# cheukwaylee/ORB_SLAM2_detailed_comments

Hardware: AMD Instinct MI355X
Metric: frames/sec ORB extract+match (1000 kp, 640x480) (higher is better)
Workload: dtype u8; 1 GPU; synthetic 640x480 mono stream, nFeatures=1000, 8 levels, scale 1.2, FAST 20/7, extract+match(t vs t-1), batch 1024 frames/GPU resident in HBM, 1 pipelines/GPU; parallelism=single GPU

## Files before the change

orb_slam2_detailed_comments_amd/csrc/orbx_kernels.hip:

```cpp
#include "orbx_device.h"
#include "orbx_inplace.h"
#include "orbx_fast_net.h"
#include "orbx_track.h"
#include "../../include/orbx_pattern_data.h"

#define L0_ROWS 8
#ifndef L0_FF
#define L0_FF 1
#endif
#ifndef RR_FF
#define RR_FF 1
#endif
#define QT_KPT ORBX_QT_KPT
#ifndef QT_DROP_STAGE_A
#define QT_DROP_STAGE_A 1
#endif
#ifndef QT_ONE_SCAN
#define QT_ONE_SCAN 1
#endif
#ifndef QT_REG_SIZE
#define QT_REG_SIZE 1
#endif
#ifndef QT_CENSUS_NODES
#define QT_CENSUS_NODES 1
// ... 1927 lines not shown
                const uint32_t a01 = __builtin_amdgcn_alignbyte(w1, w0, j), a12 = __builtin_amdgcn_alignbyte(w2, w1, j),
                               a23 = __builtin_amdgcn_alignbyte(w3, w2, j);
                hv[j] = __builtin_amdgcn_udot4(a01, KLO, __builtin_amdgcn_udot4(a12, KHI, 0u, false), false);
                hv[4 + j] = __builtin_amdgcn_udot4(a12, KLO, __builtin_amdgcn_udot4(a23, KHI, 0u, false), false);
            }
            uint4 o;
            o.x = hv[0] | (hv[1] << 16);
            o.y = hv[2] | (hv[3] << 16);
            o.z = hv[4] | (hv[5] << 16);
            o.w = hv[6] | (hv[7] << 16);
            *(uint4 *)(hrow + r * DS_HC + 8 * q8) = o;
        }
#endif
        __builtin_amdgcn_fence(__ATOMIC_RELEASE, "wavefront");
        __builtin_amdgcn_wave_barrier();
        __builtin_amdgcn_fence(__ATOMIC_ACQUIRE, "wavefront");
        if (dbg_stop == 3) return;
        const float factorPI = (float)(3.1415926535897932384626433832795 / 180.f);
        const float angle = angle_deg * factorPI;
                const OrbxSinCos sc = orbx_sincosf_pinned(angle);
        const float a = sc.c, b = sc.s;
        const int wvec = (L.pw - 2 * L.org) & ~3;
#if DS_PATTERN_F32
#define DS_PX(t) (((t) & 1) ? patf[(t) >> 1].z : patf[(t) >> 1].x)
#define DS_PY(t) (((t) & 1) ? patf[(t) >> 1].w : patf[(t) >> 1].y)
#else
        const int pw4[4] = {pat.x, pat.y, pat.z, pat.w};
#define DS_PX(t) ((float)(signed char)((pw4[(t) >> 1] >> (16 * ((t) & 1))) & 0xff))
#define DS_PY(t) ((float)(signed char)((pw4[(t) >> 1] >> (16 * ((t) & 1) + 8)) & 0xff))
#endif
        unsigned long long words[4];
        if (x + (DS_R - 3) < wvec) {
#if DS_COLFIRST
            const uint32_t cbias = (uint32_t)(2 * ((DS_R - 3) * DS_VC + (DS_R - 3))) - 0x400000u * (2u * DS_VC) - (0x4B400000u << 1);
#else
            const uint32_t cbias = (uint32_t)(2 * ((DS_R - 3) * DS_HC + (DS_R - 3))) - 0x400000u * (2u * DS_HC) - (0x4B400000u << 1);
#endif
            const uint32_t hbase = (uint32_t)(uintptr_t)(orbx_lds_u16p)hrow + cbias;
            float tv[8];
            float nb = -b;
            asm("" : "+v"(nb));
#pragma unroll
            for (int t0 = 0; t0 < 8; t0 += DS_TAP_BATCH) {
                uint32_t adr[DS_TAP_BATCH], I[DS_TAP_BATCH];
#pragma unroll
                for (int k = 0; k < DS_TAP_BATCH; ++k) {
                    const float px = DS_PX(t0 + k), py = DS_PY(t0 + k);
                    float fy, fx;
                    if (FPM == ORBX_FP_GCC_FMA) {
                        fy = __builtin_fmaf(px, b, py * a);
                        fx = __builtin_fmaf(px, a, py * nb);
                    } else {
                        fy = px * b + py * a;
                        fx = px * a + py * nb;
                    }
                    const uint32_t uy = __float_as_uint(fy + 12582912.0f), ux = __float_as_uint(fx + 12582912.0f);
#if DS_COLFIRST
#if DS_MFMA
                    uint32_t ay = (uy << 1) + hbase;
                    asm("" : "+v"(ay));
                    adr[k] = __umul24(ux, 2u * DS_VC) + ay;
#else
                    adr[k] = __umul24(uy, 2u * DS_VC) + ((ux << 1) + hbase);
#endif
#else
                    adr[k] = __umul24(uy, 2u * DS_HC) + ((ux << 1) + hbase);
                    asm("" : "+v"(adr[k]));
#endif
                }
#if DS_COLFIRST
                orbx_ds_taps<DS_TAP_BATCH>(adr, I);
#else
#pragma unroll
                for (int k = 0; k < DS_TAP_BATCH; ++k) {
                    const orbx_lds_u16p hp = (orbx_lds_u16p)(uintptr_t)adr[k];
                    const uint32_t r0 = hp[3 * DS_HC], r1 = (uint32_t)hp[2 * DS_HC] + hp[4 * DS_HC],
                                   r2 = (uint32_t)hp[1 * DS_HC] + hp[5 * DS_HC], r3 = (uint32_t)hp[0] + hp[6 * DS_HC];
                    I[k] = __umul24(55u, r0) + __umul24(49u, r1) + __umul24(34u, r2) + __umul24(18u, r3);
                }
#endif
#pragma unroll
                for (int k = 0; k < DS_TAP_BATCH; ++k) tv[t0 + k] = __builtin_fminf(__builtin_rintf((float)I[k] * (1.f / 65536.f)), 255.f);
            }
#pragma unroll
            for (int r = 0; r < 4; ++r) words[r] = orbx_ballot(tv[2 * r] < tv[2 * r + 1]);
        } else {
            int tval[8];
#pragma unroll
            for (int t0 = 0; t0 < 8; t0 += DS_TAP_BATCH) {
                uint32_t adr[DS_TAP_BATCH], I[DS_TAP_BATCH];
                int ixs[DS_TAP_BATCH];
#pragma unroll
                for (int k = 0; k < DS_TAP_BATCH; ++k) {
                    const float px = DS_PX(t0 + k), py = DS_PY(t0 + k);
                    float fy, fx;
                    if (FPM == ORBX_FP_GCC_FMA) {
                        fy = __builtin_fmaf(px, b, py * a);
                        fx = __builtin_fmaf(px, a, -(py * b));
                    } else {
                        fy = px * b + py * a;
                        fx = px * a - py * b;
                    }
                    const int iy = (int)__builtin_rintf(fy), ix = (int)__builtin_rintf(fx);
                    ixs[k] = ix;
#if DS_COLFIRST
#if DS_MFMA
                    adr[k] = (uint32_t)(uintptr_t)(orbx_lds_u16p)hrow + 2u * (uint32_t)(__mul24(ix + DS_R - 3, DS_VC) + (iy + DS_R - 3));
#else
                    adr[k] = (uint32_t)(uintptr_t)(orbx_lds_u16p)hrow + 2u * (uint32_t)(__mul24(iy + DS_R - 3, DS_VC) + (ix + DS_R - 3));
#endif
#else
                    adr[k] = (uint32_t)(__mul24(iy + DS_R - 3, DS_HC) + (ix + DS_R - 3));
#endif
                }
#if DS_COLFIRST
                orbx_ds_taps<DS_TAP_BATCH>(adr, I);
#else
#pragma unroll
                for (int k = 0; k < DS_TAP_BATCH; ++k) {
                    const uint16_t *hp = hrow + adr[k];
                    const uint32_t r0 = hp[3 * DS_HC], r1 = (uint32_t)hp[2 * DS_HC] + hp[4 * DS_HC],
                                   r2 = (uint32_t)hp[1 * DS_HC] + hp[5 * DS_HC], r3 = (uint32_t)hp[0] + hp[6 * DS_HC];
                    I[k] = __umul24(55u, r0) + __umul24(49u, r1) + __umul24(34u, r2) + __umul24(18u, r3);
                }
#endif
#pragma unroll
                for (int k = 0; k < DS_TAP_BATCH; ++k) {
                    const uint32_t tie = x + ixs[k] >= wvec ? 1u : ((I[k] >> 16) & 1u);
                    tval[t0 + k] = (int)min((I[k] + 0x7fffu + tie) >> 16, 255u);
                }
            }
#pragma unroll
            for (int r = 0; r < 4; ++r) words[r] = orbx_ballot(tval[2 * r] < tval[2 * r + 1]);
        }
        if (lane < 4) {
            unsigned long long w = lane == 0 ? words[0] : lane == 1 ? words[1] : lane == 2 ? words[2] : words[3];
            *(unsigned long long *)(desc + ((long long)f * cap + oi) * 32 + 8 * lane) = w;
        }
        if (lane == 0) {
            orbx_keypoint kp;
            float fx = (float)x, fy = (float)y;
            if (level != 0) { fx = fx * L.scale; fy = fy * L.scale; }
            kp.x = fx; kp.y = fy;
            kp.size = L.size;
            kp.angle = angle_deg;
            kp.response = (float)(pos >> 24);
            kp.octave = level;
            kp.class_id = -1;
            kps[(long long)f * cap + oi] = kp;
        }
    }
}

#define MT_SPLIT 16
#define MT_WAVES 4
#define MT_QPW(QT) (32 * (QT))
#define MT_QPB(QT) (MT_WAVES * MT_QPW(QT))
#define MT_CHUNK 4096
typedef int mt_v4i __attribute__((ext_vector_type(4)));
typedef int mt_v16i __attribute__((ext_vector_type(16)));
__device__ __forceinline__ uint32_t mt_min2(uint32_t a, uint32_t b) { return a < b ? a : b; }
__device__ __forceinline__ uint32_t mt_max2(uint32_t a, uint32_t b) { return a > b ? a : b; }
template <int QT>
__global__ __launch_bounds__(64 * MT_WAVES, QT == 2 ? 3 : 2) void k_match(const uint8_t *__restrict__ q, const int *__restrict__ nq,
                                                         long long q_stride, const uint8_t *__restrict__ t,
                                                         const int *__restrict__ nt, long long t_stride,
                                                         uint2 *__restrict__ partial, int *__restrict__ best_idx,
                                                         int *__restrict__ best_dist, int *__restrict__ second_dist,
                                                         int out_stride, int nsplit) {
    __shared__ __attribute__((aligned(16))) int s_tk[MT_CHUNK];
    const int lane = threadIdx.x & 63, w = __builtin_amdgcn_readfirstlane(threadIdx.x >> 6), pr = blockIdx.z, sp = blockIdx.y;
    const int NQ = min(nq[pr], out_stride), NT = min(nt[pr], 1 << 20);
    if ((int)blockIdx.x * MT_QPB(QT) >= NQ) return;
    const int r = lane & 31, h = lane >> 5;
    const uint8_t *qp = q + (long long)pr * q_stride;
    const uint8_t *tp = t + (long long)pr * t_stride;
    const int per = ((NT + 31) / 32 + nsplit - 1) / nsplit * 32;
    const int j0 = min(NT, sp * per), j1 = min(NT, j0 + per);
    const int qw = blockIdx.x * MT_QPB(QT) + w * MT_QPW(QT);
    const bool wave_on = qw < NQ;
    mt_v4i bq[QT][8];
    int pq[QT];
#pragma unroll
    for (int c = 0; c < QT; ++c) {
        const int qi = qw + 32 * c + r;
        uint4 v = make_uint4(0, 0, 0, 0);
        if (qi < NQ) v = *(const uint4 *)(qp + (long long)qi * 32 + 16 * h);
        pq[c] = __popc(v.x) + __popc(v.y) + __popc(v.z) + __popc(v.w);
        pq[c] += __shfl_xor(pq[c], 32);
#pragma unroll
        for (int p = 0; p < 8; ++p) {
            bq[c][p][0] = (int)((v.x << (7 - p)) & 0x80808080u);
            bq[c][p][1] = (int)((v.y << (7 - p)) & 0x80808080u);
            bq[c][p][2] = (int)((v.z << (7 - p)) & 0x80808080u);
            bq[c][p][3] = (int)((v.w << (7 - p)) & 0x80808080u);
        }
    }
    uint32_t gbest[QT], gsecond[QT];
#pragma unroll
    for (int c = 0; c < QT; ++c) gbest[c] = gsecond[c] = 0xffffffffu;
    for (int c0 = j0; c0 < j1; c0 += MT_CHUNK) {
        const int c1 = min(j1, c0 + MT_CHUNK), n = c1 - c0, npad = (n + 31) & ~31;
        __syncthreads();
        for (int i = threadIdx.x; i < npad; i += 64 * MT_WAVES) {
            int key = 0x7fffffff;
            if (i < n) {
                const uint4 a = *(const uint4 *)(tp + (long long)(c0 + i) * 32), b = *(const uint4 *)(tp + (long long)(c0 + i) * 32 + 16);
                const int pt = __popc(a.x) + __popc(a.y) + __popc(a.z) + __popc(a.w) + __popc(b.x) + __popc(b.y) + __popc(b.z) + __popc(b.w);
                key = ((pt + 256) << 12) | i;
            }
            s_tk[i] = key;
        }
        __syncthreads();
        if (!wave_on) continue;
        int best[QT], second[QT];
#pragma unroll
        for (int c = 0; c < QT; ++c) best[c] = second[c] = 0x7fffffff;
        const uint8_t *trow = tp + (long long)(c0 + r) * 32 + 16 * h;
        uint4 ta = make_uint4(0, 0, 0, 0);
        if (r < n) ta = *(const uint4 *)trow;
        for (int jt = 0; jt < npad; jt += 32) {
            const uint4 tc = ta;
            ta = make_uint4(0, 0, 0, 0);
            if (jt + 32 + r < n) ta = *(const uint4 *)(trow + (long long)(jt + 32) * 32);
            mt_v16i acc[QT];
            {
                const int4 *kp = (const int4 *)(s_tk + jt + 4 * h);
#pragma unroll
                for (int g = 0; g < 4; ++g) {
                    const int4 k4 = kp[2 * g];
                    acc[0][4 * g] = k4.x; acc[0][4 * g + 1] = k4.y; acc[0][4 * g + 2] = k4.z; acc[0][4 * g + 3] = k4.w;
                }
#pragma unroll
                for (int c = 1; c < QT; ++c) acc[c] = acc[0];
            }
#pragma unroll
            for (int p = 0; p < 8; ++p) {
                mt_v4i a;
                if (p < 6) {
                    a[0] = (int)((tc.x << (6 - p)) & 0x40404040u); a[1] = (int)((tc.y << (6 - p)) & 0x40404040u);
                    a[2] = (int)((tc.z << (6 - p)) & 0x40404040u); a[3] = (int)((tc.w << (6 - p)) & 0x40404040u);
                } else if (p == 6) {
                    a[0] = (int)(tc.x & 0x40404040u); a[1] = (int)(tc.y & 0x40404040u);
                    a[2] = (int)(tc.z & 0x40404040u); a[3] = (int)(tc.w & 0x40404040u);
                } else {
                    a[0] = (int)((tc.x >> 1) & 0x40404040u); a[1] = (int)((tc.y >> 1) & 0x40404040u);
                    a[2] = (int)((tc.z >> 1) & 0x40404040u); a[3] = (int)((tc.w >> 1) & 0x40404040u);
                }
#pragma unroll
                for (int c = 0; c < QT; ++c) acc[c] = __builtin_amdgcn_mfma_i32_32x32x32_i8(a, bq[c][p], acc[c], 0, 0, 0);
            }
#pragma unroll
            for (int i = 0; i < 16; ++i) {
#pragma unroll
                for (int c = 0; c < QT; ++c) {
                    const int kc = acc[c][i];
                    second[c] = max(min(best[c], second[c]), min(max(best[c], second[c]), kc));
                    best[c] = min(best[c], kc);
                }
            }
        }
#pragma unroll
        for (int c = 0; c < QT; ++c) {
            const uint32_t b = best[c] == 0x7fffffff ? 0xffffffffu
                                                     : ((uint32_t)((best[c] >> 12) + pq[c] - 256) << 20) | (uint32_t)(c0 + (best[c] & 4095));
            const uint32_t s2 = second[c] == 0x7fffffff ? 0xffffffffu
                                                        : ((uint32_t)((second[c] >> 12) + pq[c] - 256) << 20) | (uint32_t)(c0 + (second[c] & 4095));
            gsecond[c] = mt_min2(mt_min2(gsecond[c], s2), mt_max2(gbest[c], b));
            gbest[c] = mt_min2(gbest[c], b);
        }
    }
    if (!wave_on) return;
#pragma unroll
    for (int c = 0; c < QT; ++c) {
        const uint32_t ob = (uint32_t)__shfl_xor((int)gbest[c], 32), os = (uint32_t)__shfl_xor((int)gsecond[c], 32);
        const uint32_t second = mt_min2(mt_min2(gsecond[c], os), mt_max2(gbest[c], ob));
        const uint32_t best = mt_min2(gbest[c], ob);
        const int qi = qw + 32 * c + r;
        if (h == 0 && qi < NQ) {
            if (nsplit > 1) {
                partial[((long long)pr * nsplit + sp) * out_stride + qi] = make_uint2(best, second);
            } else {
                const long long o = (long long)pr * out_stride + qi;
                best_idx[o] = best == 0xffffffffu ? -1 : (int)(best & 0xfffffu);
                best_dist[o] = best == 0xffffffffu ? 0x7fffffff : (int)(best >> 20);
                second_dist[o] = second == 0xffffffffu ? 0x7fffffff : (int)(second >> 20);
            }
        }
    }
}

typedef int mt_v8i __attribute__((ext_vector_type(8)));
typedef float mt_v16f __attribute__((ext_vector_type(16)));
#define MT_F4_NONE 0x7f7fffff
#ifndef MT_F4_LB2
#define MT_F4_LB2 3
#endif
#ifndef MT_F4_LB4
#define MT_F4_LB4 2
#endif
#ifndef MT_F4_USE4
#define MT_F4_USE4 1
#endif
template <int QT>
__global__ __launch_bounds__(64 * MT_WAVES, QT == 2 ? MT_F4_LB2 : MT_F4_LB4) void k_match_f4(const uint8_t *__restrict__ q, const int *__restrict__ nq,
                                                         long long q_stride, const uint8_t *__restrict__ t,
                                                         const int *__restrict__ nt, long long t_stride,
                                                         uint2 *__restrict__ partial, int *__restrict__ best_idx,
                                                         int *__restrict__ best_dist, int *__restrict__ second_dist,
                                                         int out_stride, int nsplit) {
    __shared__ __attribute__((aligned(16))) float s_tk[MT_CHUNK];
    const int lane = threadIdx.x & 63, w = __builtin_amdgcn_readfirstlane(threadIdx.x >> 6), pr = blockIdx.z, sp = blockIdx.y;
    const int NQ = min(nq[pr], out_stride), NT = min(nt[pr], 1 << 20);
    if ((int)blockIdx.x * MT_QPB(QT) >= NQ) return;
    const int r = lane & 31, h = lane >> 5;
    const uint8_t *qp = q + (long long)pr * q_stride;
    const uint8_t *tp = t + (long long)pr * t_stride;
    const int per = ((NT + 31) / 32 + nsplit - 1) / nsplit * 32;
    const int j0 = min(NT, sp * per), j1 = min(NT, j0 + per);
    const int qw = blockIdx.x * MT_QPB(QT) + w * MT_QPW(QT);
    const bool wave_on = qw < NQ;
    mt_v4i bq[QT][4];
    int pq[QT];
#pragma unroll
    for (int c = 0; c < QT; ++c) {
        const int qi = qw + 32 * c + r;
        uint4 v = make_uint4(0, 0, 0, 0);
        if (qi < NQ) v = *(const uint4 *)(qp + (long long)qi * 32 + 16 * h);
        pq[c] = __popc(v.x) + __popc(v.y) + __popc(v.z) + __popc(v.w);
        pq[c] += __shfl_xor(pq[c], 32);
        const uint32_t vv[4] = {v.x, v.y, v.z, v.w};
#pragma unroll
        for (int p = 0; p < 4; ++p) {
#pragma unroll
            for (int k = 0; k < 4; ++k) {
                const uint32_t e = (vv[p] >> k) & 0x11111111u;
                bq[c][p][k] = (int)((e << 1) | (e << 2) | (e << 3));
            }
        }
    }
    uint32_t gbest[QT], gsecond[QT];
#pragma unroll
    for (int c = 0; c < QT; ++c) gbest[c] = gsecond[c] = 0xffffffffu;
    for (int c0 = j0; c0 < j1; c0 += MT_CHUNK) {
        const int c1 = min(j1, c0 + MT_CHUNK), n = c1 - c0, npad = (n + 31) & ~31;
        __syncthreads();
        for (int i = threadIdx.x; i < npad; i += 64 * MT_WAVES) {
            float key = __int_as_float(MT_F4_NONE);
            if (i < n) {
                const uint4 a = *(const uint4 *)(tp + (long long)(c0 + i) * 32), b = *(const uint4 *)(tp + (long long)(c0 + i) * 32 + 16);
                const int pt = __popc(a.x) + __popc(a.y) + __popc(a.z) + __popc(a.w) + __popc(b.x) + __popc(b.y) + __popc(b.z) + __popc(b.w);
                key = (float)(((pt + 256) << 12) | i);
            }
            s_tk[i] = key;
        }
        __syncthreads();
        if (!wave_on) continue;
        int best[QT], second[QT];
#pragma unroll
        for (int c = 0; c < QT; ++c) best[c] = second[c] = MT_F4_NONE;
        const uint8_t *trow = tp + (long long)(c0 + r) * 32 + 16 * h;
        uint4 ta = make_uint4(0, 0, 0, 0);
        if (r < n) ta = *(const uint4 *)trow;
        for (int jt = 0; jt < npad; jt += 32) {
            const uint4 tc = ta;
            ta = make_uint4(0, 0, 0, 0);
            if (jt + 32 + r < n) ta = *(const uint4 *)(trow + (long long)(jt + 32) * 32);
            mt_v16f acc[QT];
            {
                const float4 *kp = (const float4 *)(s_tk + jt + 4 * h);
#pragma unroll
                for (int g = 0; g < 4; ++g) {
                    const float4 k4 = kp[2 * g];
                    acc[0][4 * g] = k4.x; acc[0][4 * g + 1] = k4.y; acc[0][4 * g + 2] = k4.z; acc[0][4 * g + 3] = k4.w;
                }
#pragma unroll
                for (int c = 1; c < QT; ++c) acc[c] = acc[0];
            }
            const uint32_t tw[4] = {tc.x, tc.y, tc.z, tc.w};
#pragma unroll
            for (int p = 0; p < 4; ++p) {
                mt_v8i a = {0, 0, 0, 0, 0, 0, 0, 0};
                a[0] = (int)((tw[p] << 2) & 0x44444444u); a[1] = (int)((tw[p] << 1) & 0x44444444u);
                a[2] = (int)(tw[p] & 0x44444444u);        a[3] = (int)((tw[p] >> 1) & 0x44444444u);
#pragma unroll
                for (int c = 0; c < QT; ++c) {
                    mt_v8i b = {0, 0, 0, 0, 0, 0, 0, 0};
                    b[0] = bq[c][p][0]; b[1] = bq[c][p][1]; b[2] = bq[c][p][2]; b[3] = bq[c][p][3];
                    acc[c] = __builtin_amdgcn_mfma_scale_f32_32x32x64_f8f6f4(a, b, acc[c], 4, 4, 0, 137, 0, 127);
                }
            }
#pragma unroll
            for (int i = 0; i < 16; ++i) {
#pragma unroll
                for (int c = 0; c < QT; ++c) {
                    const int kc = __float_as_int(acc[c][i]);
                    second[c] = max(min(best[c], second[c]), min(max(best[c], second[c]), kc));
                    best[c] = min(best[c], kc);
                }
            }
        }
#pragma unroll
        for (int c = 0; c < QT; ++c) {
            const int bk = (int)__int_as_float(best[c]), sk = (int)__int_as_float(second[c]);
            const uint32_t b = best[c] == MT_F4_NONE ? 0xffffffffu
                                                     : ((uint32_t)((bk >> 12) + pq[c] - 256) << 20) | (uint32_t)(c0 + (bk & 4095));
            const uint32_t s2 = second[c] == MT_F4_NONE ? 0xffffffffu
                                                        : ((uint32_t)((sk >> 12) + pq[c] - 256) << 20) | (uint32_t)(c0 + (sk & 4095));
            gsecond[c] = mt_min2(mt_min2(gsecond[c], s2), mt_max2(gbest[c], b));
            gbest[c] = mt_min2(gbest[c], b);
        }
    }
    if (!wave_on) return;
#pragma unroll
    for (int c = 0; c < QT; ++c) {
        const uint32_t ob = (uint32_t)__shfl_xor((int)gbest[c], 32), os = (uint32_t)__shfl_xor((int)gsecond[c], 32);
        const uint32_t second = mt_min2(mt_min2(gsecond[c], os), mt_max2(gbest[c], ob));
        const uint32_t best = mt_min2(gbest[c], ob);
        const int qi = qw + 32 * c + r;
        if (h == 0 && qi < NQ) {
            if (nsplit > 1) {
                partial[((long long)pr * nsplit + sp) * out_stride + qi] = make_uint2(best, second);
            } else {
                const long long o = (long long)pr * out_stride + qi;
                best_idx[o] = best == 0xffffffffu ? -1 : (int)(best & 0xfffffu);
                best_dist[o] = best == 0xffffffffu ? 0x7fffffff : (int)(best >> 20);
                second_dist[o] = second == 0xffffffffu ? 0x7fffffff : (int)(second >> 20);
            }
        }
    }
}

__global__ __launch_bounds__(64) void k_match_valu(const uint8_t *__restrict__ q, const int *__restrict__ nq,
                                                         long long q_stride, const uint8_t *__restrict__ t,
                                                         const int *__restrict__ nt, long long t_stride,
                                                         uint2 *__restrict__ partial, int out_stride, int nsplit) {
    const int lane = threadIdx.x, pr = blockIdx.z, sp = blockIdx.y;
    const int NQ = min(nq[pr], out_stride), NT = min(nt[pr], 1 << 20);
    const int qw = blockIdx.x * 128;
    if (qw >= NQ) return;
    const int qi0 = qw + lane, qi1 = qi0 + 64;
    const uint4 *qp = (const uint4 *)(q + (long long)pr * q_stride);
    const uint4 *tp = (const uint4 *)(t + (long long)pr * t_stride);
    uint4 qa0 = make_uint4(0, 0, 0, 0), qb0 = qa0, qa1 = qa0, qb1 = qa0;
    if (qi0 < NQ) { qa0 = qp[2 * qi0]; qb0 = qp[2 * qi0 + 1]; }
    if (qi1 < NQ) { qa1 = qp[2 * qi1]; qb1 = qp[2 * qi1 + 1]; }
    const int chunk = (NT + nsplit - 1) / nsplit;
    const int j0 = sp * chunk, j1 = min(NT, j0 + chunk);
    uint32_t best0 = 0xffffffffu, second0 = 0xffffffffu, best1 = 0xffffffffu, second1 = 0xffffffffu;
#pragma unroll 4
    for (int j = j0; j < j1; ++j) {
        const uint4 ta = tp[2 * j], tb = tp[2 * j + 1];
        const uint32_t d0 = __popc(qa0.x ^ ta.x) + __popc(qa0.y ^ ta.y) + __popc(qa0.z ^ ta.z) + __popc(qa0.w ^ ta.w) +
                            __popc(qb0.x ^ tb.x) + __popc(qb0.y ^ tb.y) + __popc(qb0.z ^ tb.z) + __popc(qb0.w ^ tb.w);
        const uint32_t d1 = __popc(qa1.x ^ ta.x) + __popc(qa1.y ^ ta.y) + __popc(qa1.z ^ ta.z) + __popc(qa1.w ^ ta.w) +
                            __popc(qb1.x ^ tb.x) + __popc(qb1.y ^ tb.y) + __popc(qb1.z ^ tb.z) + __popc(qb1.w ^ tb.w);
        const uint32_t key0 = (d0 << 20) | (uint32_t)j, key1 = (d1 << 20) | (uint32_t)j;
        second0 = max(min(best0, second0), min(max(best0, second0), key0));
        best0 = min(best0, key0);
        second1 = max(min(best1, second1), min(max(best1, second1), key1));
        best1 = min(best1, key1);
    }
    uint2 *po = partial + ((long long)pr * nsplit + sp) * out_stride;
    if (qi0 < NQ) po[qi0] = make_uint2(best0, second0);
    if (qi1 < NQ) po[qi1] = make_uint2(best1, second1);
}

__global__ __launch_bounds__(256) void k_match_merge(const int *__restrict__ nq, const uint2 *__restrict__ partial,
                                                     int *__restrict__ best_idx, int *__restrict__ best_dist,
                                                     int *__restrict__ second_dist, int out_stride, int nsplit) {
    const int pr = blockIdx.y, qi = blockIdx.x * 256 + threadIdx.x;
    if (qi >= min(nq[pr], out_stride)) return;
    uint32_t best = 0xffffffffu, second = 0xffffffffu;
    for (int k = 0; k < nsplit; ++k) {
        const uint2 p = partial[((long long)pr * nsplit + k) * out_stride + qi];
        second = min(min(second, p.y), max(best, p.x));
        best = min(best, p.x);
    }
    const long long o = (long long)pr * out_stride + qi;
    best_idx[o] = best == 0xffffffffu ? -1 : (int)(best & 0xfffffu);
    best_dist[o] = best == 0xffffffffu ? 0x7fffffff : (int)(best >> 20);
    second_dist[o] = second == 0xffffffffu ? 0x7fffffff : (int)(second >> 20);
}

__global__ __launch_bounds__(256) void k_hamming_matrix(const uint8_t *__restrict__ q, int nq,
                                                        const uint8_t *__restrict__ t, int nt,
                                                        uint16_t *__restrict__ dist) {
    const long long i = (long long)blockIdx.x * 256 + threadIdx.x;
    if (i >= (long long)nq * nt) return;
    const int qi = (int)(i / nt), ti = (int)(i - (long long)qi * nt);
    const uint4 *qp = (const uint4 *)q + 2 * qi, *tp = (const uint4 *)t + 2 * ti;
    const uint4 qa = qp[0], qb = qp[1], ta = tp[0], tb = tp[1];
    dist[i] = (uint16_t)(__popc(qa.x ^ ta.x) + __popc(qa.y ^ ta.y) + __popc(qa.z ^ ta.z) + __popc(qa.w ^ ta.w) +
                         __popc(qb.x ^ tb.x) + __popc(qb.y ^ tb.y) + __popc(qb.z ^ tb.z) + __popc(qb.w ^ tb.w));
}

__device__ __forceinline__ uint32_t st_row16_min(uint32_t v) {
    v = min(v, (uint32_t)__builtin_amdgcn_update_dpp((int)v, (int)v, 0x121, 0xf, 0xf, false));
    v = min(v, (uint32_t)__builtin_amdgcn_update_dpp((int)v, (int)v, 0x122, 0xf, 0xf, false));
    v = min(v, (uint32_t)__builtin_amdgcn_update_dpp((int)v, (int)v, 0x124, 0xf, 0xf, false));
    v = min(v, (uint32_t)__builtin_amdgcn_update_dpp((int)v, (int)v, 0x128, 0xf, 0xf, false));
    return v;
}
__device__ __forceinline__ uint32_t st_row16_sum(uint32_t v) {
    v += (uint32_t)__builtin_amdgcn_update_dpp((int)v, (int)v, 0x121, 0xf, 0xf, false);
    v += (uint32_t)__builtin_amdgcn_update_dpp((int)v, (int)v, 0x122, 0xf, 0xf, false);
    v += (uint32_t)__builtin_amdgcn_update_dpp((int)v, (int)v, 0x124, 0xf, 0xf, false);
    v += (uint32_t)__builtin_amdgcn_update_dpp((int)v, (int)v, 0x128, 0xf, 0xf, false);
    return v;
}
#define ST_KPB 16
__device__ __forceinline__ void orbx_stereo_body(const OrbxStereoGeom &sg, const orbx_keypoint *__restrict__ kL,
                                                 const uint8_t *__restrict__ dL, int nL,
                                                 const orbx_keypoint *__restrict__ kR,
                                                 const uint8_t *__restrict__ dR, int nR,
                                                 const uint8_t *__restrict__ pyrL, const uint8_t *__restrict__ pyrR,
                                                 float *__restrict__ uRight, float *__restrict__ depth,
                                                 int *__restrict__ sad, const int *__restrict__ row_begin,
                                                 const uint2 *__restrict__ row_items) {
    const int l16 = threadIdx.x & 15;
    const int iL = blockIdx.x * ST_KPB + (threadIdx.x >> 4);
    bool act = iL < nL;
    float uL = 0.f, vL = 0.f;
    int levelL = 0;
    if (act) { const orbx_keypoint kp = kL[iL]; uL = kp.x; vL = kp.y; levelL = kp.octave; }
    if (act && l16 == 0) { uRight[iL] = -1.0f; depth[iL] = -1.0f; sad[iL] = -1; }
    const long long row = (long long)vL;
    act = act && row >= 0 && row < sg.nrows0;
    const float maxD = sg.mbf / sg.mb, minD = 0.f;
    const float minU = uL - maxD, maxU = uL - minD;
    act = act && !(maxU < 0);
    uint4 qa = make_uint4(0, 0, 0, 0), qb = qa;
    if (act) { const uint4 *qp = (const uint4 *)(dL + (long long)iL * 32); qa = qp[0]; qb = qp[1]; }
    uint32_t best = 0xffffffffu;
    if (row_begin) {
        int j = 0, j1 = 0;
        if (act) { j = row_begin[row] + l16; j1 = row_begin[row + 1]; }
        for (; j < j1; j += 16) {
            const uint2 it = row_items[j];
            const int iR = (int)(it.y & 0xffffu), octR = (int)(it.y >> 16);
            const float xR = __uint_as_float(it.x);
            const bool cand = (int)(octR >= levelL - 1) & (int)(octR <= levelL + 1) & (int)(xR >= minU) & (int)(xR <= maxU);
            if (cand) {
                const uint4 *tp = (const uint4 *)(dR + (long long)iR * 32);
                const uint4 ta = tp[0], tb = tp[1];
                const uint32_t d = __popc(qa.x ^ ta.x) + __popc(qa.y ^ ta.y) + __popc(qa.z ^ ta.z) + __popc(qa.w ^ ta.w) +
                                   __popc(qb.x ^ tb.x) + __popc(qb.y ^ tb.y) + __popc(qb.z ^ tb.z) + __popc(qb.w ^ tb.w);
                if (d < 100u) best = min(best, (d << 16) | (uint32_t)iR);
            }
        }
    } else {
        for (int iR = act ? l16 : nR; iR < nR; iR += 16) {
            const orbx_keypoint kr = kR[iR];
            const float r = 2.0f * sg.scale[kr.octave];
            const int maxr = (int)ceilf(kr.y + r), minr = (int)floorf(kr.y - r);
            const bool cand = (int)(row >= minr) & (int)(row <= maxr) & (int)(kr.octave >= levelL - 1) &
                              (int)(kr.octave <= levelL + 1) & (int)(kr.x >= minU) & (int)(kr.x <= maxU);
            if (cand) {
                const uint4 *tp = (const uint4 *)(dR + (long long)iR * 32);
                const uint4 ta = tp[0], tb = tp[1];
                const uint32_t d = __popc(qa.x ^ ta.x) + __popc(qa.y ^ ta.y) + __popc(qa.z ^ ta.z) + __popc(qa.w ^ ta.w) +
                                   __popc(qb.x ^ tb.x) + __popc(qb.y ^ tb.y) + __popc(qb.z ^ tb.z) + __popc(qb.w ^ tb.w);
                if (d < 100u) best = min(best, (d << 16) | (uint32_t)iR);
            }
        }
    }
    best = st_row16_min(best);
    act = act && best != 0xffffffffu && (best >> 16) < 75u;
    const int bestIdxR = act ? (int)(best & 0xffffu) : 0;
    float uR0 = 0.f;
    if (act) uR0 = kR[bestIdxR].x;
    const float scaleFactor = sg.inv_scale[levelL];
    const float scaleduL = roundf(uL * scaleFactor), scaledvL = roundf(vL * scaleFactor);
    const float scaleduR0 = roundf(uR0 * scaleFactor);
    const int w = 5, Lh = 5;
    const int W = sg.pw[levelL], H = sg.ph[levelL], pitch = sg.pitch[levelL];
    const int y0 = (int)(scaledvL - w), x0 = (int)(scaleduL - w);
    act = act && !(y0 < 0 || y0 + 2 * w + 1 > H || x0 < 0 || x0 + 2 * w + 1 > W);
    const float iniu = scaleduR0 - Lh - w, endu = scaleduR0 + Lh + w + 1;
    act = act && !(iniu < 0 || endu >= W);
    uint32_t acc[11];
#pragma unroll
    for (int s = 0; s < 11; ++s) acc[s] = 0u;
    if (act) {
        const uint8_t *IL = pyrL + sg.off[levelL] + (long long)y0 * pitch + x0;
        const uint8_t *IR = pyrR + sg.off[levelL] + (long long)y0 * pitch + ((int)scaleduR0 - w);
        const uint32_t cL = IL[w * pitch + w];
        const orbx_uint3_u cw = *(const orbx_uint3_u *)(IR + w * pitch);
        uint32_t Cs[11];
#pragma unroll
        for (int s = 0; s < 11; ++s) {
            const uint32_t cwd = s < 4 ? cw.x : s < 8 ? cw.y : cw.z;
            Cs[s] = (((cwd >> (8 * (s & 3))) & 0xffu) + 511u - cL) * 0x10001u;
        }
#pragma unroll
        for (int k = 0; k < 4; ++k) {
            int q0 = l16 + 16 * k, q1 = q0 + 64;
            if (q1 >= 121) q1 = 60;
            const int y_0 = q0 / 11, x_0 = q0 - 11 * y_0, y_1 = q1 / 11, x_1 = q1 - 11 * y_1;
            const uint32_t L0 = IL[y_0 * pitch + x_0], L1 = IL[y_1 * pitch + x_1];
            const orbx_uint3_u r0 = *(const orbx_uint3_u *)(IR + y_0 * pitch + x_0 - Lh);
            const orbx_uint3_u r1 = *(const orbx_uint3_u *)(IR + y_1 * pitch + x_1 - Lh);
            const uint32_t A0 = L0 | (L1 << 16);
#pragma unroll
            for (int s = 0; s < 11; ++s) {
                const uint32_t lo = s < 4 ? r0.x : s < 8 ? r0.y : r0.z, hi = s < 4 ? r1.x : s < 8 ? r1.y : r1.z;
                const uint32_t sel = (uint32_t)(s & 3) | (0x0cu << 8) | ((uint32_t)(4 + (s & 3)) << 16) | (0x0cu << 24);
                const uint32_t B = __builtin_amdgcn_perm(hi, lo, sel) + 0x01ff01ffu;
                acc[s] = __builtin_amdgcn_sad_u16(A0 + Cs[s], B, acc[s]);
            }
        }
    }
#pragma unroll
    for (int s = 0; s < 11; ++s) acc[s] = st_row16_sum(acc[s]);
    if (!act || l16 != 0) return;
    int bestDistS = 0x7fffffff, bestinc = 0;
#pragma unroll
    for (int s = 0; s < 11; ++s)
        if ((int)acc[s] < bestDistS) { bestDistS = (int)acc[s]; bestinc = s - Lh; }
    if (bestinc == -Lh || bestinc == Lh) return;
    float dist1 = 0.f, dist2 = 0.f, dist3 = 0.f;
#pragma unroll
    for (int s = 1; s < 10; ++s)
        if (s - Lh == bestinc) { dist1 = (float)(int)acc[s - 1]; dist2 = (float)(int)acc[s]; dist3 = (float)(int)acc[s + 1]; }
    const float deltaR = (dist1 - dist3) / (2.0f * (dist1 + dist3 - 2.0f * dist2));
    if (deltaR < -1 || deltaR > 1) return;
    float bestuR = sg.scale[levelL] * ((float)scaleduR0 + (float)bestinc + deltaR);
    float disparity = uL - bestuR;
    if (disparity >= minD && disparity < maxD) {
        if (disparity <= 0) { disparity = (float)0.01; bestuR = (float)((double)uL - 0.01); }
        depth[iL] = sg.mbf / disparity;
        uRight[iL] = bestuR;
        sad[iL] = bestDistS;
    }
}

__global__ __launch_bounds__(256) void k_stereo(OrbxStereoGeom sg, const orbx_keypoint *__restrict__ kL,
                                                const uint8_t *__restrict__ dL, int nL,
                                                const orbx_keypoint *__restrict__ kR,
                                                const uint8_t *__restrict__ dR, int nR,
                                                const uint8_t *__restrict__ pyrL, const uint8_t *__restrict__ pyrR,
                                                float *__restrict__ uRight, float *__restrict__ depth,
                                                int *__restrict__ sad, const int *__restrict__ row_begin,
                                                const uint2 *__restrict__ row_items) {
    orbx_stereo_body(sg, kL, dL, nL, kR, dR, nR, pyrL, pyrR, uRight, depth, sad, row_begin, row_items);
}
__global__ __launch_bounds__(256) void k_stereo_batch(OrbxStereoGeom sg, const orbx_keypoint *__restrict__ kL,
                                                      const uint8_t *__restrict__ dL, const int *__restrict__ nL,
                                                      const orbx_keypoint *__restrict__ kR,
                                                      const uint8_t *__restrict__ dR, const int *__restrict__ nR, int cap,
                                                      const uint8_t *__restrict__ pyrL, const uint8_t *__restrict__ pyrR,
                                                      long long pyr_bytes, float *__restrict__ uRight,
                                                      float *__restrict__ depth, int *__restrict__ sad,
                                                      const int *__restrict__ row_begin, const uint2 *__restrict__ row_items,
                                                      int items_per_pair) {
    const long long p = blockIdx.y;
    orbx_stereo_body(sg, kL + p * cap, dL + p * cap * 32, min(nL[p], cap), kR + p * cap, dR + p * cap * 32, min(nR[p], cap),
                     pyrL + p * pyr_bytes, pyrR + p * pyr_bytes, uRight + p * cap, depth + p * cap, sad + p * cap,
                     row_begin ? row_begin + p * (sg.nrows0 + 1) : nullptr, row_items ? row_items + p * items_per_pair : nullptr);
}
#define ST_MAX_ROWS 4096
__global__ __launch_bounds__(1024) void k_stereo_rows(OrbxStereoGeom sg, const orbx_keypoint *__restrict__ kR,
                                                      const int *__restrict__ nR, int cap, int *__restrict__ row_begin,
                                                      uint2 *__restrict__ row_items, int items_per_pair, int n_direct) {
    __shared__ int s_cnt[ST_MAX_ROWS + 1];
    __shared__ int s_part[1024];
    const long long p = blockIdx.x;
    const int t = threadIdx.x, n = nR ? min(nR[p], cap) : n_direct, rows = sg.nrows0;
    const orbx_keypoint *k = kR + p * cap;
    for (int i = t; i <= rows; i += 1024) s_cnt[i] = 0;
    __syncthreads();
    for (int i = t; i < n; i += 1024) {
        const float r = 2.0f * sg.scale[k[i].octave];
        const int maxr = min((int)ceilf(k[i].y + r), rows - 1), minr = max((int)floorf(k[i].y - r), 0);
        for (int y = minr; y <= maxr; ++y) atomicAdd(&s_cnt[y], 1);
    }
    __syncthreads();
    const int chunk = (rows + 1023) / 1024, r0 = t * chunk, r1 = min(r0 + chunk, rows);
    int sum = 0;
    for (int y = r0; y < r1; ++y) sum += s_cnt[y];
    s_part[t] = sum;
    __syncthreads();
    for (int o = 1; o < 1024; o <<= 1) {
        const int v = t >= o ? s_part[t - o] : 0;
        __syncthreads();
        s_part[t] += v;
        __syncthreads();
    }
    int run = s_part[t] - sum;
    int *rb = row_begin + p * (rows + 1);
    for (int y = r0; y < r1; ++y) { const int c = s_cnt[y]; s_cnt[y] = run; rb[y] = run; run += c; }
    if (t == 1023) rb[rows] = s_part[1023];
    __syncthreads();
    uint2 *items = row_items + p * items_per_pair;
    for (int i = t; i < n; i += 1024) {
        const float r = 2.0f * sg.scale[k[i].octave];
        const int maxr = min((int)ceilf(k[i].y + r), rows - 1), minr = max((int)floorf(k[i].y - r), 0);
        for (int y = minr; y <= maxr; ++y) {
            const int pos = atomicAdd(&s_cnt[y], 1);
            if (pos < items_per_pair) items[pos] = make_uint2(__float_as_uint(k[i].x), (uint32_t)i | ((uint32_t)k[i].octave << 16));
        }
    }
}
__global__ __launch_bounds__(256) void k_stereo_cut(const int *__restrict__ nL, int cap, const int *__restrict__ sad,
// ... 1829 lines not shown
```

Baseline: 411,000 frames/s.

## Software-pipeline f4 matcher MFMA with min-reduction across query halves

Restructures the k_match_f4 inner loop so MFMAs for one half of the query tiles are interleaved with best/second-min updates of the other half, using explicit scheduling group barriers. Train descriptor loads switch to buffer loads with a range-limited resource, which removes the per-lane bounds checks. The min-update is paired to process two candidates per step, reducing the VALU op count. The aim is to hide MFMA latency behind VALU reduction work, at the cost of more live registers and fragile scheduling hints.

```diff
diff --git a/orb_slam2_detailed_comments_amd/csrc/orbx_kernels.hip b/orb_slam2_detailed_comments_amd/csrc/orbx_kernels.hip
--- a/orb_slam2_detailed_comments_amd/csrc/orbx_kernels.hip
+++ b/orb_slam2_detailed_comments_amd/csrc/orbx_kernels.hip
@@ -2253,6 +2253,61 @@
 #ifndef MT_F4_USE4
 #define MT_F4_USE4 1
 #endif
+#ifndef MT_F4_PAIR
+#define MT_F4_PAIR 2
+#endif
+#ifndef MT_F4_ROTATE
+#define MT_F4_ROTATE 3
+#endif
+__device__ __forceinline__ void mt_f4_update2(int &best, int &second, int k1, int k2) {
+    const int s3 = max(min(k1, k2), min(max(k1, k2), best));
+#if MT_F4_PAIR == 2
+    asm("" : "+v"(k1));
+#endif
+    best = min(min(best, k1), k2);
+    second = min(second, s3);
+}
+__device__ __forceinline__ void mt_f4_update4(int &best, int &second, const mt_v16f &acc, int i0) {
+#if MT_F4_PAIR
+    mt_f4_update2(best, second, __float_as_int(acc[i0]), __float_as_int(acc[i0 + 1]));
+    mt_f4_update2(best, second, __float_as_int(acc[i0 + 2]), __float_as_int(acc[i0 + 3]));
+#else
+#pragma unroll
+    for (int i = i0; i < i0 + 4; ++i) {
+        const int kc = __float_as_int(acc[i]);
+        second = max(min(best, second), min(max(best, second), kc));
+        best = min(best, kc);
+    }
+#endif
+}
+__device__ __forceinline__ mt_v16f mt_f4_mfma(const mt_v4i &a4, const mt_v4i &b4, const mt_v16f &c) {
+    const mt_v8i a = {a4[0], a4[1], a4[2], a4[3], 0, 0, 0, 0}, b = {b4[0], b4[1], b4[2], b4[3], 0, 0, 0, 0};
+    return __builtin_amdgcn_mfma_scale_f32_32x32x64_f8f6f4(a, b, c, 4, 4, 0, 137, 0, 127);
+}
+__device__ __forceinline__ void mt_f4_expand1(mt_v4i &a, const uint4 &tc, int p) {
+    const uint32_t w = p == 0 ? tc.x : p == 1 ? tc.y : p == 2 ? tc.z : tc.w;
+    a[0] = (int)((w << 2) & 0x44444444u); a[1] = (int)((w << 1) & 0x44444444u);
+    a[2] = (int)(w & 0x44444444u);        a[3] = (int)((w >> 1) & 0x44444444u);
+}
+__device__ __forceinline__ mt_v16f mt_f4_keys(const float *tile) {
+    mt_v16f k;
+#pragma unroll
+    for (int g = 0; g < 4; ++g) {
+        const float4 k4 = ((const float4 *)tile)[2 * g];
+        k[4 * g] = k4.x; k[4 * g + 1] = k4.y; k[4 * g + 2] = k4.z; k[4 * g + 3] = k4.w;
+    }
+    return k;
+}
+typedef unsigned int mt_v4u __attribute__((ext_vector_type(4)));
+__device__ __forceinline__ uint4 mt_f4_tload(__amdgpu_buffer_rsrc_t rs, int off) {
+    const mt_v4u v = __builtin_amdgcn_raw_buffer_load_b128(rs, off, 0, 0);
+    return make_uint4(v.x, v.y, v.z, v.w);
+}
+#define MT_F4_STEP_END(G, C0) do { \
+        for (int c_ = (C0); c_ < (C0) + (G); ++c_) asm volatile("" : "+v"(best[c_]), "+v"(second[c_])); \
+        for (int g_ = 0; g_ < (G); ++g_) { __builtin_amdgcn_sched_group_barrier(0x8, 1, 0); __builtin_amdgcn_sched_group_barrier(0x2, MT_F4_STEP_VALU, 0); } \
+        __builtin_amdgcn_sched_barrier(0); } while (0)
+#define MT_F4_STEP_VALU (MT_F4_PAIR ? 10 : 12)
 template <int QT>
 __global__ __launch_bounds__(64 * MT_WAVES, QT == 2 ? MT_F4_LB2 : MT_F4_LB4) void k_match_f4(const uint8_t *__restrict__ q, const int *__restrict__ nq,
                                                          long long q_stride, const uint8_t *__restrict__ t,
@@ -2310,13 +2365,68 @@
         int best[QT], second[QT];
 #pragma unroll
         for (int c = 0; c < QT; ++c) best[c] = second[c] = MT_F4_NONE;
+#if MT_F4_ROTATE & 1
+        const __amdgpu_buffer_rsrc_t trs = __builtin_amdgcn_make_buffer_rsrc((void *)(tp + (long long)c0 * 32), 0, n * 32, 0x00020000);
+        const int toff = r * 32 + 16 * h;
+#define MT_F4_TLOAD(j) mt_f4_tload(trs, toff + (j) * 32)
+#else
         const uint8_t *trow = tp + (long long)(c0 + r) * 32 + 16 * h;
+#define MT_F4_TLOAD(j) ((j) + r < n ? *(const uint4 *)(trow + (long long)(j) * 32) : make_uint4(0, 0, 0, 0))
+#endif
+#if MT_F4_ROTATE & 2
+        constexpr int G = QT / 2;
+        mt_v4i ax[4];
+        uint4 ta = MT_F4_TLOAD(0);
+#pragma unroll
+        for (int p = 0; p < 4; ++p) mt_f4_expand1(ax[p], ta, p);
+        ta = MT_F4_TLOAD(32);
+        mt_v16f keys = mt_f4_keys(s_tk + 4 * h);
+        mt_v16f acc[QT];
+#pragma unroll
+        for (int c = G; c < QT; ++c)
+#pragma unroll
+            for (int i = 0; i < 16; ++i) acc[c][i] = __int_as_float(MT_F4_NONE);
+        for (int jt = 0; jt < npad; jt += 32) {
+#pragma unroll
+            for (int p = 0; p < 4; ++p) {
+#pragma unroll
+                for (int c = 0; c < G; ++c) acc[c] = mt_f4_mfma(ax[p], bq[c][p], p == 0 ? keys : acc[c]);
+#pragma unroll
+                for (int c = G; c < QT; ++c) mt_f4_update4(best[c], second[c], acc[c], 4 * p);
+                MT_F4_STEP_END(G, G);
+            }
+#pragma unroll
+            for (int p = 0; p < 4; ++p) {
+#pragma unroll
+                for (int c = G; c < QT; ++c) acc[c] = mt_f4_mfma(ax[p], bq[c][p], p == 0 ? keys : acc[c]);
+                if (p == 1) { asm volatile("" :: "v"(keys)); keys = mt_f4_keys(s_tk + min(jt + 32, npad - 32) + 4 * h); }
+                if (p >= 1) mt_f4_expand1(ax[p - 1], ta, p - 1);
+#pragma unroll
+                for (int c = 0; c < G; ++c) mt_f4_update4(best[c], second[c], acc[c], 4 * p);
+                MT_F4_STEP_END(G, 0);
+            }
+            mt_f4_expand1(ax[3], ta, 3);
+            ta = MT_F4_TLOAD(jt + 64);
+        }
+#pragma unroll
+        for (int c = G; c < QT; ++c)
+#pragma unroll
+            for (int p = 0; p < 4; ++p) mt_f4_update4(best[c], second[c], acc[c], 4 * p);
+#else
+#if MT_F4_ROTATE & 1
+        uint4 ta = MT_F4_TLOAD(0);
+#else
         uint4 ta = make_uint4(0, 0, 0, 0);
         if (r < n) ta = *(const uint4 *)trow;
+#endif
         for (int jt = 0; jt < npad; jt += 32) {
             const uint4 tc = ta;
+#if MT_F4_ROTATE & 1
+            ta = MT_F4_TLOAD(jt + 32);
+#else
             ta = make_uint4(0, 0, 0, 0);
             if (jt + 32 + r < n) ta = *(const uint4 *)(trow + (long long)(jt + 32) * 32);
+#endif
             mt_v16f acc[QT];
             {
                 const float4 *kp = (const float4 *)(s_tk + jt + 4 * h);
@@ -2341,6 +2451,13 @@
                     acc[c] = __builtin_amdgcn_mfma_scale_f32_32x32x64_f8f6f4(a, b, acc[c], 4, 4, 0, 137, 0, 127);
                 }
             }
+#if MT_F4_PAIR
+#pragma unroll
+            for (int i = 0; i < 16; i += 2) {
+#pragma unroll
+                for (int c = 0; c < QT; ++c) mt_f4_update2(best[c], second[c], __float_as_int(acc[c][i]), __float_as_int(acc[c][i + 1]));
+            }
+#else
 #pragma unroll
             for (int i = 0; i < 16; ++i) {
 #pragma unroll
@@ -2350,7 +2467,10 @@
                     best[c] = min(best[c], kc);
                 }
             }
-        }
+#endif
+        }
+#endif
+#undef MT_F4_TLOAD
 #pragma unroll
         for (int c = 0; c < QT; ++c) {
             const int bk = (int)__int_as_float(best[c]), sk = (int)__int_as_float(second[c]);
```

New measurement: 414,400 frames/s (median of 6 runs). Within noise of the previous version (+0.8%).
